# INK-USC/RE-Net

Measured on NVIDIA H100. Metric: rgcn_aggregate_edge_messages_per_sec, higher is better.
Workload: dtype f32

## Files before the change

renet_b200/csrc/common.cuh:

```cuda
#pragma once
#include <cuda_runtime.h>
#include <stdint.h>
#include <stdio.h>
#include <stdarg.h>

#include "../../include/renet_b200.h"

namespace renet {

void set_error(const char* fmt, ...);
void count_launch(int n = 1);
void note_gemm_kernel(int kernel);
int last_gemm_kernel();

#define RENET_CHECK_ARG(cond, ...)                  \
  do {                                              \
    if (!(cond)) {                                  \
      ::renet::set_error(__VA_ARGS__);              \
      return RENET_ERR_INVALID_ARG;                 \
    }                                               \
  } while (0)

#define RENET_CHECK_CUDA(expr)                                                        \
  do {                                                                                \
    cudaError_t _e = (expr);                                                          \
    if (_e != cudaSuccess) {                                                          \
      ::renet::set_error("%s failed: %s (%s:%d)", #expr, cudaGetErrorString(_e),     \
                         __FILE__, __LINE__);                                         \
      return RENET_ERR_CUDA;                                                          \
    }                                                                                 \
  } while (0)

#define RENET_CHECK_LAUNCH(name)                                                      \
  do {                                                                                \
    cudaError_t _e = cudaGetLastError();                                              \
    if (_e != cudaSuccess) {                                                          \
      ::renet::set_error("launch of %s failed: %s", name, cudaGetErrorString(_e));    \
      return RENET_ERR_CUDA;                                                          \
    }                                                                                 \
    ::renet::count_launch();                                                          \
  } while (0)

constexpr int kNumSMs = 132;

__device__ __forceinline__ float4 ldg_f4(const float* p) {
  return __ldg(reinterpret_cast<const float4*>(p));
}
__device__ __forceinline__ float4 ldg_f4_stream(const float* p) {
  float4 r;
  asm volatile("ld.global.nc.L1::no_allocate.v4.f32 {%0,%1,%2,%3}, [%4];"
               : "=f"(r.x), "=f"(r.y), "=f"(r.z), "=f"(r.w)
               : "l"(p));
  return r;
}
__device__ __forceinline__ void st_f4(float* p, float4 v) { *reinterpret_cast<float4*>(p) = v; }

__device__ __forceinline__ void red_add_f4(float* p, float4 v) {
  asm volatile("red.global.add.v4.f32 [%0], {%1,%2,%3,%4};" ::"l"(p), "f"(v.x), "f"(v.y), "f"(v.z),
               "f"(v.w)
               : "memory");
}

bool deterministic();
int set_deterministic(int on);
int det_scratch(int64_t bytes, cudaStream_t stream, void** out);
int launch_sum_partials(const float* parts, int n_parts, int64_t stride, int64_t rows, int cols, float* out, int64_t ldo,
                        bool accumulate, cudaStream_t stream);
int scatter_add_rows_det(const float* src, int64_t ld, const int32_t* index, const int32_t* outer, float* dst, int64_t n_rows,
                         int d, cudaStream_t stream);

int sgemm_nn(const float* A, const int32_t* a_index, int64_t lda, const float* B, int64_t ldb, float* C,
             int64_t ldc, const float* bias, int64_t M, int32_t N, int32_t K, bool accumulate,
             cudaStream_t stream);
bool sgemm_nn_tiled_ok(const float* A, int64_t lda, const float* B, int64_t ldb, const float* C, int64_t ldc,
                       const float* bias, int32_t N, int32_t K);
int sgemm_nn_ffma(const float* A, const int32_t* a_index, int64_t lda, const float* B, int64_t ldb, float* C,
// ... 67 lines not shown
```

renet_b200/csrc/rgcn_fwd.cu:

```cuda
#include <stdlib.h>

#include "common.cuh"
#include "rgcn_tile.cuh"
#include "rgcn_stream.cuh"

namespace renet {
namespace {

template <bool RELU, bool HAS_LOOP, bool INDEXED, int NODES = kTileNodes>
__global__ void __launch_bounds__(kTileWarps * 32, 768 / (kTileWarps * 32))
rgcn_gather_d200_kernel(const float* __restrict__ H, const int32_t* __restrict__ h_index,
                        const float* __restrict__ W, const int32_t* __restrict__ row_ptr,
                        const int32_t* __restrict__ col_src, const int32_t* __restrict__ col_type,
                        const float* __restrict__ norm, float* __restrict__ Hout, int N, int passthrough) {
  __shared__ __align__(16) float agg[NODES][200];
  __shared__ __align__(16) float loopbuf[HAS_LOOP ? NODES : 1][200];
  __shared__ __align__(16) float head[kTileWarps][200];
  __shared__ int head_mask[NODES];
  __shared__ float normbuf[NODES];
  __shared__ int s_rp[NODES + 1];
  const int tid = threadIdx.x;
  const int v0 = blockIdx.x * NODES;
  const int nv = min(NODES, N - v0);
  tile_prefetch_epilogue(loopbuf, normbuf, Hout + (int64_t)v0 * 200, norm + v0, nv, HAS_LOOP, tid, kTileWarps * 32);
// ... 65 lines not shown
    else if (e && e[0] == 's') v = 3;
  }
  return v;
}
bool gather_use_stream(int64_t E, int64_t N, bool indexed_input) {
  const int c = gather_kernel_choice();
  const int64_t min_nodes = indexed_input ? kStreamMinNodes : kStreamMinPlainNodes;
  return c == 3 || (c == 0 && E >= kStreamMinEdges && N >= min_nodes && N <= kStreamMaxNodes);
}

static long long* g_stream_dbg = nullptr;
void set_stream_debug_buffer(long long* p) { g_stream_dbg = p; }

int stream_cfg_choice() {
  static int v = -1;
  if (v < 0) {
    const char* e = getenv("RENET_STREAM_CFG");
    v = e ? atoi(e) : 0;
  }
  return v;
}

template <bool RELU, bool HAS_LOOP, bool INDEXED, class Cfg>
static int launch_stream_cfg(const float* H, const int32_t* h_index, const float* W, const int32_t* row_ptr,
                             const int32_t* col_src, const int32_t* col_type, const float* norm, float* Hout, int N, int R2,
                             const int32_t* hot_rel, int n_hot, int E_hint, cudaStream_t stream) {
  static bool attr_done = false;
  if (!attr_done) {
    RENET_CHECK_CUDA(cudaFuncSetAttribute(rgcn_gather_stream_kernel<RELU, HAS_LOOP, INDEXED, false, Cfg>,
                                          cudaFuncAttributeMaxDynamicSharedMemorySize, Cfg::kSmemBytes));
    attr_done = true;
  }
  long long* dbg = g_stream_dbg;
  rgcn_gather_stream_kernel<RELU, HAS_LOOP, INDEXED, false, Cfg><<<kNumSMs, Cfg::kThreads, Cfg::kSmemBytes, stream>>>(
      H, h_index, W, row_ptr, col_src, col_type, norm, Hout, N, R2, hot_rel, n_hot, E_hint, dbg);
  RENET_CHECK_LAUNCH("rgcn_gather_stream_kernel");
  return RENET_OK;
}

template <bool RELU, bool HAS_LOOP, bool INDEXED>
static int launch_stream(const float* H, const int32_t* h_index, const float* W, const int32_t* row_ptr,
                         const int32_t* col_src, const int32_t* col_type, const float* norm, float* Hout, int N, int R2,
                         const int32_t* hot_rel, int n_hot, int E_hint, cudaStream_t stream) {
#define RENET_ST(...) return launch_stream_cfg<RELU, HAS_LOOP, INDEXED, __VA_ARGS__>(H, h_index, W, row_ptr, col_src, col_type, norm, Hout, N, R2, hot_rel, n_hot, E_hint, stream)
  if (RELU && HAS_LOOP) {
    switch (stream_cfg_choice()) {
      case 1: RENET_ST(StCfg<28, 2, 31, false>);
      case 2: RENET_ST(StCfg<24, 2, 44, false>);
      default: break;
    }
  }
  RENET_ST(StDefault<false>);
#undef RENET_ST
}

int launch_rgcn_gather(const float* H, const int32_t* h_index, const float* W, const int32_t* row_ptr,
                       const int32_t* col_src, const int32_t* col_type, const float* norm, float* Hout,
                       int64_t N, int64_t E, int d_in, int d_out, int nb, int relu, int has_loop,
                       cudaStream_t stream, int R2, const int32_t* hot_rel, int n_hot) {
  if (N == 0) return RENET_OK;
  const int passthrough = (E == 0) ? 1 : 0;
  const bool fast = d_in == 200 && d_out == 200 && nb == 100 &&
                    ((reinterpret_cast<uintptr_t>(H) | reinterpret_cast<uintptr_t>(W) |
                      reinterpret_cast<uintptr_t>(Hout)) & 15) == 0;
  if (fast) {
    const int key = (relu ? 4 : 0) | (has_loop ? 2 : 0) | (h_index ? 1 : 0);
    if (!passthrough && gather_use_stream(E, N, h_index != nullptr)) {
#define RENET_LAUNCH_STREAM(R, L, I) return launch_stream<R, L, I>(H, h_index, W, row_ptr, col_src, col_type, norm, Hout, (int)N, R2, hot_rel, n_hot, (int)E, stream)
      switch (key) {
        case 0: RENET_LAUNCH_STREAM(false, false, false);
// ... 37 lines not shown
```

renet_b200/csrc/rgcn_stream.cuh:

```cuda
#pragma once
#include <type_traits>

#include "common.cuh"
#include "umma.cuh"

namespace renet {

constexpr int kStRpCap = 1024;
constexpr int kStMaxR2 = 2048;
constexpr int kStNodeCost = 2;
constexpr int kStSlot = 800;
constexpr int kStHotGroups = 8;
template <int WARPS, int D, int HOT, bool BWD>
struct StCfg {
  static constexpr int kWarps = WARPS, kThreads = WARPS * 32, kD = D, kHot = HOT;
  static constexpr int kHotPerGroup = (HOT + kStHotGroups - 1) / kStHotGroups;
  static constexpr int kBlk = (32 / D) * D;
  static constexpr int kOffRing = 0;
  static constexpr int kOffHot = kOffRing + WARPS * D * kStSlot;
  static constexpr int kOffHeads = kOffHot + HOT * 1600;
  static constexpr int kOffRp = kOffHeads + WARPS * 800;
  static constexpr int kOffSlotOf = kOffRp + kStRpCap * 4;
  static constexpr int kOffIdx = kOffSlotOf + kStMaxR2;
  static constexpr int kOffSc = kOffIdx + WARPS * 64 * 8;
// ... 87 lines not shown
  auto global_timer = []() {
    long long t;
    asm volatile("mov.u64 %0, %%globaltimer;" : "=l"(t));
    return t;
  };
  if (dbg) { stamp(0, clock64()); stamp(5, global_timer()); }
  constexpr int D = Cfg::kD, kBlk = Cfg::kBlk, kStWarps = Cfg::kWarps, kStThreads = Cfg::kThreads;
  float* heads = reinterpret_cast<float*>(st_smem + Cfg::kOffHeads);
  int32_t* s_rp = reinterpret_cast<int32_t*>(st_smem + Cfg::kOffRp);
  uint8_t* slot_of = st_smem + Cfg::kOffSlotOf;
  int* flags = reinterpret_cast<int*>(st_smem + Cfg::kOffFlags);
  int* s_part = flags + kStWarps;
  int* s_e0 = s_part + 16;
  uint64_t* bars = reinterpret_cast<uint64_t*>(st_smem + Cfg::kOffBars);
  int* cnt = reinterpret_cast<int*>(st_smem + Cfg::kOffRing);
  int* hist = cnt + kStMaxR2;

  const int tid = threadIdx.x, lane = tid & 31;
  const int warp = __shfl_sync(0xffffffffu, tid >> 5, 0);
  const bool tail4 = lane < 4;
  const bool use_hot = R2 > 0 && R2 <= kStMaxR2 && Cfg::kHot > 0;
  const bool given_hot = use_hot && hot_rel != nullptr;
  {
    const int64_t gt = (int64_t)blockIdx.x * Cfg::kThreads + threadIdx.x;
    const int64_t n_rp_lines = ((int64_t)N + 1 + 31) / 32, n_e_lines = ((int64_t)E_hint + 31) / 32;
    const char* pf = nullptr;
    if (gt < n_rp_lines) pf = reinterpret_cast<const char*>(row_ptr) + gt * 128;
    else if (gt < n_rp_lines + n_e_lines) pf = reinterpret_cast<const char*>(col_a) + (gt - n_rp_lines) * 128;
    else if (gt < n_rp_lines + 2 * n_e_lines) pf = reinterpret_cast<const char*>(col_type) + (gt - n_rp_lines - n_e_lines) * 128;
    else if (INDEXED && gt < 2 * n_rp_lines + 2 * n_e_lines - 1)
      pf = reinterpret_cast<const char*>(x_index) + (gt - n_rp_lines - 2 * n_e_lines) * 128;
    if (pf) asm volatile("prefetch.global.L2 [%0];" ::"l"(pf));
  }
  const int E = __ldg(row_ptr + N);
  const int half = tid >> 8, ht = tid & 255;
  const int c_idx = blockIdx.x + half;
  const bool searching = tid < 512 && c_idx > 0 && c_idx < (int)gridDim.x;
  const int probe0 = min((ht + 1) * (N / 256 + 1) - 1, N);
  const int val0 = searching ? __ldg(row_ptr + probe0) : 0;
  constexpr int kHotIters = (Cfg::kHot + 31) / 32;
  const int n_hot_given = given_hot ? min(n_hot_arg, Cfg::kHot) : 0;
  if (warp == 1) {
    for (int sl = lane; sl < n_hot_given; sl += 32) st_cp_async4(smem_u32(hist + sl), hot_rel + sl);
    asm volatile("cp.async.commit_group;" ::: "memory");
  }
  const uint32_t hot_bar0 = smem_u32(bars + kStWarps * D);
  const uint32_t head_bar0 = hot_bar0 + kStHotGroups * 8;

  if (tid < 16) s_part[tid] = 0;
  if (tid < kStWarps) flags[tid] = 0;
  if (lane == 0) {
#pragma unroll
    for (int k = 0; k < D; ++k) mbar_init(smem_u32(bars + warp * D + k), 1);
    mbar_init(head_bar0 + warp * 8, 1);
    if (warp == 0)
      for (int gr = 0; gr < kStHotGroups; ++gr) mbar_init(hot_bar0 + gr * 8, 1);
    asm volatile("fence.mbarrier_init.release.cluster;" ::: "memory");
  }
  if (!given_hot)
    for (int i = tid; i < kStMaxR2 + 256; i += kStThreads) cnt[i] = 0;
  for (int i = tid; i < kStMaxR2 / 4; i += kStThreads) reinterpret_cast<uint32_t*>(slot_of)[i] = 0u;
  __syncthreads();
  auto load_hot = [&](int n_hot, auto row_of) {
    if (lane < kStHotGroups) {
      const int rows = min(max(n_hot - lane * Cfg::kHotPerGroup, 0), Cfg::kHotPerGroup);
      st_expect_tx(hot_bar0 + lane * 8, (uint32_t)rows * 1600u);
    }
    __syncwarp();
#pragma unroll
    for (int k = 0; k < kHotIters; ++k) {
      const int sl = lane + 32 * k;
      if (sl < n_hot)
        st_bulk_g2s(smem_u32(st_smem + Cfg::kOffHot + sl * 1600), W + (int64_t)row_of(k) * 400, 1600,
                    hot_bar0 + (sl / Cfg::kHotPerGroup) * 8);
    }
  };
  const int64_t total_cost = (int64_t)E + (int64_t)kStNodeCost * N;
  const int64_t target = ((int64_t)c_idx * total_cost) / gridDim.x;
  int lo = 0, hi = N;
  const int rounds = N < 256 ? 1 : (N < 65536 ? 2 : (N < (1 << 24) ? 3 : 4));
  for (int r = 0; r < rounds; ++r) {
    const int step = (hi - lo) / 256 + 1;
    const int p = min(lo + (ht + 1) * step - 1, hi);
    const int val = r == 0 ? val0 : (searching ? __ldg(row_ptr + p) : 0);
    const bool below = searching && (int64_t)val + (int64_t)kStNodeCost * p < target;
    const unsigned m = __ballot_sync(0xffffffffu, below);
    if (lane == 0 && m) atomicAdd(&s_part[2 * r + (half & 1)], __popc(m));
    __syncthreads();
    const int f = s_part[2 * r + (half & 1)];
    if (r == rounds - 1 && searching) {
      if (ht == f) { s_part[10 + half] = lo + f; s_part[12 + half] = val; }
      if (ht == f - 1) s_part[14 + half] = val + 1;
    }
    const int new_hi = min(lo + (f + 1) * step - 1, hi);
// ... 109 lines not shown
        const int slot = atomicAdd(&s_part[9], 1);
        slot_of[r] = (uint8_t)(slot + 1);
        hist[slot] = r;
      }
    }
    __syncthreads();
    if (thr > 1) {
      for (int r = tid; r < R2; r += kStThreads) {
        if (min(cnt[r], 255) == thr - 1) {
          const int slot = atomicAdd(&s_part[9], 1);
          if (slot < Cfg::kHot) { slot_of[r] = (uint8_t)(slot + 1); hist[slot] = r; }
        }
      }
      __syncthreads();
    }
    if (warp == 1) load_hot(min(s_part[9], Cfg::kHot), [&](int k) { return hist[lane + 32 * k]; });
  }
  block_gather(0);
  __syncthreads();
  block_stage(0);
  block_load(1);

  const uint32_t ring = st_opaque(smem_u32(st_smem + Cfg::kOffRing + warp * D * kStSlot));
  const uint32_t bar0 = st_opaque(smem_u32(bars + warp * D));
  const uint32_t idx_a = st_opaque(smem_u32(my_idx));
  auto issue = [&](int k, int slot) {
    if (st_elect_one()) {
      const uint32_t src = st_lds_u32(idx_a + (((uint32_t)k & 63u) << 3));
      const uint32_t bar = bar0 + slot * 8;
      st_expect_tx(bar, 800u);
      st_bulk_g2s(ring + slot * kStSlot, X + (int64_t)(int)src * 200, 800, bar);
    }
  };
  asm volatile("griddepcontrol.wait;" ::: "memory");
#pragma unroll
  for (int k = 0; k < D; ++k)
    if (k < n) issue(k, k);

  int va;
  {
    int l = A, h = A_next;
    while (h > l) {
      const int mid = (l + h) >> 1;
      if (rp(mid) >= e0) h = mid; else l = mid + 1;
    }
    va = l;
  }
  int cur = va;
  bool continued = false;
  if (n > 0 && rp(va) > e0) { cur = va - 1; continued = true; }
  int cur_end = cur < A_next ? rp(cur + 1) : ce;
  float acc[8];
#pragma unroll
  for (int i = 0; i < 8; ++i) acc[i] = 0.f;
  float2 lp[4];
  float nrm = 1.f;
#pragma unroll
  for (int k = 0; k < 4; ++k) lp[k] = make_float2(0.f, 0.f);
  auto fetch_dest = [&](int v) {
    if (v < A_next) {
      if (HAS_LOOP) {
#pragma unroll
        for (int k = 0; k < 4; ++k)
          if (k < 3 || tail4) lp[k] = *reinterpret_cast<const float2*>(Hout + (int64_t)v * 200 + 2 * (lane + 32 * k));
      }
      if (!BWD) nrm = __ldg(norm + v);
    }
// ... 148 lines not shown
```

renet_b200/csrc/umma_gemm.cu:

```cuda
#include "common.cuh"
#include <mutex>
#include <vector>

#include "umma.cuh"

namespace renet {
namespace {

constexpr int UM = 128;
constexpr int UN = 200;
constexpr int UNP = 208;
constexpr int UKC = 40;
constexpr int USLABS = UKC / 4;
constexpr int UTHREADS = 256;
constexpr int A_SLAB_BYTES = UM * 16;
constexpr int B_SLAB_BYTES = UNP * 16;
constexpr int A_BYTES = USLABS * A_SLAB_BYTES;
constexpr int B_BYTES = USLABS * B_SLAB_BYTES;
constexpr int STAGE_BYTES = 2 * A_BYTES + 2 * B_BYTES;
constexpr int NUM_STAGES = 2;
constexpr int SMEM_BYTES = NUM_STAGES * STAGE_BYTES;
constexpr int CLD = UNP + 4;
static_assert(UM * CLD * 4 <= SMEM_BYTES, "accumulator tile reuses the operand stages");

// ... 119 lines not shown
          o[4] += b1.x; o[5] += b1.y; o[6] += b1.z; o[7] += b1.w;
        }
        if (accumulate) {
          const float4 c0 = *reinterpret_cast<const float4*>(cp), c1 = *reinterpret_cast<const float4*>(cp + 4);
          o[0] += c0.x; o[1] += c0.y; o[2] += c0.z; o[3] += c0.w;
          o[4] += c1.x; o[5] += c1.y; o[6] += c1.z; o[7] += c1.w;
        }
        st_f4(cp, make_float4(o[0], o[1], o[2], o[3]));
        st_f4(cp + 4, make_float4(o[4], o[5], o[6], o[7]));
      }
    }
  }
}


constexpr int P_BK = 32;
constexpr int P_A_BYTES = UM * 128;
constexpr int P_B_BYTES = UNP * 128;
constexpr int P_B_CHUNK = 2 * P_B_BYTES;
constexpr int P_UN = UNP / 2;
constexpr int P_BH_BYTES = P_UN * 128;
constexpr int P_STAGE = 2 * P_A_BYTES + 2 * P_BH_BYTES;
constexpr int P_THREADS = 384;
constexpr int P_CLD = P_UN + 4;
__host__ __device__ constexpr int p_stages(int epi) { return epi == 0 ? 3 : 2; }
__host__ __device__ constexpr int p_staging_bytes(int epi) { return epi == 0 ? 0 : 2 * 64 * P_CLD * 4; }
__host__ __device__ constexpr int p_smem(int epi) { return p_stages(epi) * P_STAGE + p_staging_bytes(epi) + 1024 + 128; }
static_assert(p_smem(0) <= 232448 && p_smem(1) <= 232448, "one CTA's shared memory");
static_assert(P_STAGE % 1024 == 0 && P_BH_BYTES % 1024 == 0, "swizzle atoms stay 1024-byte aligned");

__global__ void __launch_bounds__(256)
umma_pack_b_kernel(const float* __restrict__ B, int64_t sk, int64_t sn, int N, int K, uint8_t* __restrict__ Bp,
                   int n_chunks, int tile_offset) {
  const int nt = blockIdx.x, kc = blockIdx.y;
  const int n0 = nt * UN, k0 = kc * P_BK;
  const int tile_n = min(UN, N - n0);
  uint8_t* dst = Bp + (size_t)((nt + tile_offset) * n_chunks + kc) * P_B_CHUNK;
  for (int task = blockIdx.z * 256 + threadIdx.x; task < UNP * 8; task += 256 * gridDim.z) {
    const int j = task / UNP, n = task % UNP;
    float v[4];
#pragma unroll
    for (int i = 0; i < 4; ++i) {
      const int k = k0 + 4 * j + i;
      v[i] = (n < tile_n && k < K) ? __ldg(B + (int64_t)k * sk + (int64_t)(n0 + n) * sn) : 0.f;
    }
    float4 hi, lo;
    split4(make_float4(v[0], v[1], v[2], v[3]), hi, lo);
    const uint32_t off = sw128_offset(n, j);
    *reinterpret_cast<float4*>(dst + off) = hi;
    *reinterpret_cast<float4*>(dst + P_B_BYTES + off) = lo;
  }
}

struct PUnit {
  int64_t row_base;
  int nt, half, zb, split, c_begin, n_local;
};
__device__ __forceinline__ PUnit p_unit(int64_t u, int64_t n_rt, int n_tiles, int n_chunks, int k_splits) {
  PUnit w;
  const int64_t rest = u / n_rt;
  w.row_base = (u - rest * n_rt) * UM;
  const int nh = (int)(rest % (2 * n_tiles)), z = (int)(rest / (2 * n_tiles));
  w.nt = nh >> 1;
  w.half = nh & 1;
  w.zb = z / k_splits;
  w.split = z - w.zb * k_splits;
// ... 352 lines not shown
      if (n_gt) atomicAdd(rc, n_gt);
      if (n_eq) atomicAdd(rc + 1, n_eq);
#pragma unroll
      for (int j = 0; j < 2; ++j)
        if (j < n_lists) {
          if (m_gt[j]) atomicAdd(rc + 2 + 2 * j, m_gt[j]);
          if (m_eq[j]) atomicAdd(rc + 3 + 2 * j, m_eq[j]);
        }
    }
    if (FWD && gr < M) {
      const int64_t pi = (int64_t)(w.nt * 2 + w.half) * M + gr;
      epi.pmax[pi] = run_m;
      epi.psum[pi] = run_s;
      if (SOFT) {
        epi.pdot[pi] = run_pz;
        epi.pmass[pi] = run_p;
      }
    }
  }
  ts.finish(1);
}

constexpr int R_MAX_CHUNKS = 7;
constexpr int R_CHUNK = 2 * P_BH_BYTES;
constexpr int R_THREADS = 384;
constexpr int R_SMEM = R_MAX_CHUNKS * R_CHUNK + 1024 + 8 * R_MAX_CHUNKS;
static_assert(R_SMEM <= 232448, "one CTA's shared memory");

template <bool INDEXED>
__global__ void __launch_bounds__(R_THREADS, 1)
umma_gemm_resident_kernel(const float* __restrict__ A, const int32_t* __restrict__ a_index, int64_t lda,
                          const uint8_t* __restrict__ Bp, float* __restrict__ C, int64_t ldc, const float* __restrict__ bias,
                          int64_t M, const int32_t* __restrict__ m_dev, int N, int K, int n_chunks, int accumulate,
                          int64_t batch_a, int64_t batch_bp, int64_t batch_c, int n_panels, long long* dbg) {
  extern __shared__ uint8_t smem_raw[];
  const uint32_t raw = smem_u32(smem_raw);
  const uint32_t sb = raw + ((1024 - (raw & 1023)) & 1023);
  const uint32_t bar0 = sb + R_MAX_CHUNKS * R_CHUNK;
  const int tid = threadIdx.x;
  const int wg = __shfl_sync(0xffffffffu, tid >> 7, 0);
  if (m_dev != nullptr) M = *m_dev;
  const int G = gridDim.x, b = blockIdx.x;
  const int p = (int)(((int64_t)(b + 1) * n_panels - 1) / G);
  const int cta0 = (int)((int64_t)p * G / n_panels), ncta = (int)((int64_t)(p + 1) * G / n_panels) - cta0;
  const int64_t n_rt = (M + 63) / 64;
  const int64_t t_begin = (int64_t)(b - cta0) * n_rt / ncta, t_end = (int64_t)(b - cta0 + 1) * n_rt / ncta;
  if (t_begin == t_end) return;
  const int n_tiles = (N + UN - 1) / UN;
  const int half = p & 1, nt = (p >> 1) % n_tiles, zb = (p >> 1) / n_tiles;
  GemmStamps ts(dbg, wg);
  if (tid == 0) {
    for (int c = 0; c < n_chunks; ++c) mbar_init(bar0 + 8 * c, 1);
    asm volatile("fence.mbarrier_init.release.cluster;" ::: "memory");
    const uint8_t* src = Bp + zb * batch_bp + (size_t)nt * n_chunks * P_B_CHUNK + half * P_BH_BYTES;
    for (int c = 0; c < n_chunks; ++c) {
      const uint32_t bar = bar0 + 8 * c, dst = sb + c * R_CHUNK;
      mbar_expect_tx(bar, R_CHUNK);
      bulk_copy_g2s(dst, src + (size_t)c * P_B_CHUNK, P_BH_BYTES, bar);
      bulk_copy_g2s(dst + P_BH_BYTES, src + (size_t)c * P_B_CHUNK + P_B_BYTES, P_BH_BYTES, bar);
      mbar_arrive(bar);
    }
  }
  __syncthreads();

  const int wt = tid & 127, lane = tid & 31, tig = lane & 3;
  const int ra = 16 * (wt >> 5) + (lane >> 2);
  const float* Az = A + zb * batch_a;
  auto row_ptr = [&](int64_t gr) -> const float* {
    return gr < M ? Az + (INDEXED ? (int64_t)__ldg(a_index + gr) : gr) * lda : nullptr;
  };
  auto load = [&](float (&v)[16], const float* pa, const float* pb, int c) {
#pragma unroll
    for (int j = 0; j < 8; ++j) {
      const int k = c * P_BK + 4 * j + tig;
      v[j] = (pa != nullptr && k < K) ? __ldg(pa + k) : 0.f;
      v[8 + j] = (pb != nullptr && k < K) ? __ldg(pb + k) : 0.f;
    }
  };
  int64_t t = t_begin + wg;
  const float *pa = nullptr, *pb = nullptr;
  float v[16];
  if (t < t_end) {
    pa = row_ptr(t * 64 + ra);
    pb = row_ptr(t * 64 + ra + 8);
    load(v, pa, pb, 0);
  }
  const int n0 = nt * UN, cb = half * P_UN, tile_n = min(UN, N - n0);
  float* Cz = C + zb * batch_c;
  const float* bz = bias != nullptr ? bias + zb * (int64_t)N : nullptr;
  float acc[P_UN / 2];
  for (; t < t_end; t += 3) {
    ++ts.items;
    for (int c = 0; c < n_chunks; ++c) {
      long long t0 = ts.now();
      uint32_t hi[16], lo[16];
// ... 19 lines not shown
      const uint32_t b_hi = sb + c * R_CHUNK, b_lo = b_hi + P_BH_BYTES;
      wgmma_fence();
#pragma unroll
      for (int ks = 0; ks < P_BK / 8; ++ks) {
        if (ks < nks) {
          const uint64_t dBh = make_desc_sw128(b_hi + ks * 32), dBl = make_desc_sw128(b_lo + ks * 32);
          const int j = 2 * ks;
          wgmma_tf32_n104_rs(acc, hi[j], hi[8 + j], hi[j + 1], hi[9 + j], dBh, (c | ks) != 0);
          wgmma_tf32_n104_rs(acc, lo[j], lo[8 + j], lo[j + 1], lo[9 + j], dBh, 1);
          wgmma_tf32_n104_rs(acc, hi[j], hi[8 + j], hi[j + 1], hi[9 + j], dBl, 1);
        }
      }
      wgmma_commit();
      t0 = ts.now();
      wgmma_wait<0>();
      ts.mma += ts.now() - t0;
      acc_fence(acc);
      reg_fence(hi);
      reg_fence(lo);
    }
    const long long t0 = ts.now();
    store_fragment(acc, Cz, ldc, bz, t * 64, M, n0, cb, tile_n, accumulate, wt);
    ts.epi += ts.now() - t0;
  }
  ts.finish(2);
}

__device__ __forceinline__ uint32_t dedup_hash(uint32_t v, int bits) { return (v * 0x9E3779B1u) >> (32 - bits); }

__global__ void __launch_bounds__(256)
dedup_insert_kernel(const int32_t* __restrict__ a_index, int64_t M, unsigned long long* __restrict__ table, int bits,
                    uint32_t epoch, int32_t* __restrict__ slot_row, int32_t* __restrict__ uniq, int32_t* __restrict__ link,
                    int32_t* __restrict__ count) {
  const int64_t n = (int64_t)blockIdx.x * blockDim.x + threadIdx.x;
  if (n >= M) return;
  const uint32_t v = (uint32_t)__ldg(a_index + n);
  const unsigned long long key = ((unsigned long long)epoch << 32) | v;
  const uint32_t mask = (1u << bits) - 1;
  uint32_t s = dedup_hash(v, bits);
  for (;;) {
    const unsigned long long cur = __ldcg(table + s);
    if (cur == key) break;
    if ((uint32_t)(cur >> 32) == epoch) {
      s = (s + 1) & mask;
      continue;
    }
    if (atomicCAS(table + s, cur, key) == cur) {
      const int32_t u = atomicAdd(count, 1);
      uniq[u] = (int32_t)v;
      slot_row[s] = u;
      break;
    }
  }
  link[n] = (int32_t)s;
}

__global__ void __launch_bounds__(256)
dedup_expand_kernel(const float* __restrict__ P, const int32_t* __restrict__ slot_row, const int32_t* __restrict__ link,
                    float* __restrict__ C, int64_t ldc, int64_t M, int N, int32_t* __restrict__ count) {
  if (blockIdx.x == 0 && threadIdx.x == 0) *count = 0;
  const int64_t n = ((int64_t)blockIdx.x * blockDim.x + threadIdx.x) >> 5;
  if (n >= M) return;
  const int64_t u = __ldg(slot_row + __ldg(link + n));
  const float* src = P + u * N;
  float* dst = C + n * ldc;
  for (int j = 4 * (threadIdx.x & 31); j < N; j += 128) st_f4(dst + j, ldg_f4(src + j));
// ... 30 lines not shown
  *hit = false;
  std::lock_guard<std::mutex> lk(g_pack_mu);
  if (g_weight_generation < 0 || nkeys > 6) return nullptr;
  int dev = 0;
  if (cudaGetDevice(&dev) != cudaSuccess) return nullptr;
  for (auto& e : g_pack_entries) {
    if (e.device != dev || e.nkeys != nkeys || e.bytes != bytes) continue;
    bool same = true;
    for (int i = 0; i < nkeys; ++i) same &= e.keys[i] == keys[i];
    if (!same) continue;
    *hit = e.gen == g_weight_generation;
    e.gen = g_weight_generation;
    return e.buf;
  }
  if (g_pack_entries.size() >= 64) {
    cudaFree(g_pack_entries.front().buf);
    g_pack_entries.erase(g_pack_entries.begin());
  }
  PackEntry e{};
  e.device = dev; e.nkeys = nkeys; e.bytes = bytes; e.gen = g_weight_generation;
  for (int i = 0; i < nkeys; ++i) e.keys[i] = keys[i];
  if (cudaMalloc(&e.buf, (size_t)bytes) != cudaSuccess) { cudaGetLastError(); return nullptr; }
  g_pack_entries.push_back(e);
  return e.buf;
}

int64_t umma_packed_bytes(int N, int K) {
  return (int64_t)((N + UN - 1) / UN) * ((K + P_BK - 1) / P_BK) * P_B_CHUNK;
}
bool umma_shape_ok(int N, int K) { return (K % 4 == 0) && (N % 8 == 0) && N > 0 && K > 0; }

int umma_pack_b(const float* B, int64_t sk, int64_t sn, int N, int K, void* Bp, int tile_offset, cudaStream_t stream) {
  const int n_tiles = (N + UN - 1) / UN, n_chunks = (K + P_BK - 1) / P_BK;
  umma_pack_b_kernel<<<dim3(n_tiles, n_chunks, 7), 256, 0, stream>>>(B, sk, sn, N, K, (uint8_t*)Bp, n_chunks, tile_offset);
  RENET_CHECK_LAUNCH("umma_pack_b_kernel");
  return RENET_OK;
}

static bool resident_ok(int N, int K, int batch) {
  return (K + P_BK - 1) / P_BK <= R_MAX_CHUNKS && batch * ((N + UN - 1) / UN) * 2 <= kNumSMs;
}

static int launch_resident(const float* A, const int32_t* a_index, int64_t lda, const void* Bp, float* C, int64_t ldc,
                           const float* bias, int64_t M, const int32_t* m_dev, int N, int K, bool accumulate, int batch,
                           int64_t batch_a, int64_t batch_bp, int64_t batch_c, cudaStream_t stream) {
  static bool attr_r = false;
  if (!attr_r) {
    RENET_CHECK_CUDA(cudaFuncSetAttribute(umma_gemm_resident_kernel<true>, cudaFuncAttributeMaxDynamicSharedMemorySize, R_SMEM));
    RENET_CHECK_CUDA(cudaFuncSetAttribute(umma_gemm_resident_kernel<false>, cudaFuncAttributeMaxDynamicSharedMemorySize, R_SMEM));
    attr_r = true;
  }
  const int n_chunks = (K + P_BK - 1) / P_BK, n_panels = batch * ((N + UN - 1) / UN) * 2;
  const int64_t n_work = (int64_t)n_panels * ((M + 63) / 64);
  const unsigned grid = (unsigned)(n_work < kNumSMs ? n_work : kNumSMs);
  if (a_index)
    umma_gemm_resident_kernel<true><<<grid, R_THREADS, R_SMEM, stream>>>(A, a_index, lda, (const uint8_t*)Bp, C, ldc, bias, M,
                                                                        m_dev, N, K, n_chunks, accumulate, batch_a, batch_bp,
                                                                        batch_c, n_panels, g_gemm_dbg);
  else
    umma_gemm_resident_kernel<false><<<grid, R_THREADS, R_SMEM, stream>>>(A, a_index, lda, (const uint8_t*)Bp, C, ldc, bias, M,
                                                                         m_dev, N, K, n_chunks, accumulate, batch_a, batch_bp,
                                                                         batch_c, n_panels, g_gemm_dbg);
  RENET_CHECK_LAUNCH("umma_gemm_resident_kernel");
  note_gemm_kernel(RENET_GEMM_RESIDENT);
  return RENET_OK;
}

static int launch_streaming(const float* A, const int32_t* a_index, int64_t lda, const void* Bp, float* C, int64_t ldc,
                            const float* bias, int64_t M, int N, int K, bool accumulate, int batch, int64_t batch_a,
                            int64_t batch_bp, int64_t batch_c, int epi_mode, const EpiArgs& epi, int k_splits, int64_t split_c,
                            cudaStream_t stream) {
  static bool attr2 = false;
  if (!attr2) {
    RENET_CHECK_CUDA(cudaFuncSetAttribute(umma_gemm_packed_kernel<true, 0>, cudaFuncAttributeMaxDynamicSharedMemorySize, p_smem(0)));
    RENET_CHECK_CUDA(cudaFuncSetAttribute(umma_gemm_packed_kernel<false, 0>, cudaFuncAttributeMaxDynamicSharedMemorySize, p_smem(0)));
    RENET_CHECK_CUDA(cudaFuncSetAttribute(umma_gemm_packed_kernel<false, 1>, cudaFuncAttributeMaxDynamicSharedMemorySize, p_smem(1)));
    RENET_CHECK_CUDA(cudaFuncSetAttribute(umma_gemm_packed_kernel<false, 2>, cudaFuncAttributeMaxDynamicSharedMemorySize, p_smem(2)));
    RENET_CHECK_CUDA(cudaFuncSetAttribute(umma_gemm_packed_kernel<false, 3>, cudaFuncAttributeMaxDynamicSharedMemorySize, p_smem(3)));
    RENET_CHECK_CUDA(cudaFuncSetAttribute(umma_gemm_packed_kernel<false, 4>, cudaFuncAttributeMaxDynamicSharedMemorySize, p_smem(4)));
    RENET_CHECK_CUDA(cudaFuncSetAttribute(umma_gemm_packed_kernel<false, 5>, cudaFuncAttributeMaxDynamicSharedMemorySize, p_smem(5)));
    RENET_CHECK_CUDA(cudaFuncSetAttribute(umma_gemm_packed_kernel<false, 6>, cudaFuncAttributeMaxDynamicSharedMemorySize, p_smem(6)));
    RENET_CHECK_CUDA(cudaFuncSetAttribute(umma_gemm_packed_kernel<false, 7>, cudaFuncAttributeMaxDynamicSharedMemorySize, p_smem(7)));
    attr2 = true;
  }
  const int n_tiles = (N + UN - 1) / UN, n_chunks = (K + P_BK - 1) / P_BK;
  const int64_t n_units = (M + UM - 1) / UM * (2 * n_tiles) * batch * k_splits;
  const unsigned grid = (unsigned)(n_units < kNumSMs ? n_units : kNumSMs);
#define RENET_UMMA_LAUNCH(IDX, EP)                                                                                       \
  umma_gemm_packed_kernel<IDX, EP><<<grid, P_THREADS, p_smem(EP), stream>>>(A, a_index, lda, (const uint8_t*)Bp, C, ldc, bias, \
                                                                           M, N, K, n_chunks, accumulate, batch_a, batch_bp,  \
                                                                           batch_c, epi, k_splits, split_c, n_units, \
                                                                           g_gemm_dbg)
  if (epi_mode == 1) RENET_UMMA_LAUNCH(false, 1);
  else if (epi_mode == 2) RENET_UMMA_LAUNCH(false, 2);
  else if (epi_mode == 3) RENET_UMMA_LAUNCH(false, 3);
  else if (epi_mode == 4) RENET_UMMA_LAUNCH(false, 4);
// ... 84 lines not shown
  }
  if (M > w->rows) {
    if (w->ix) RENET_CHECK_CUDA(cudaFreeAsync(w->ix, stream));
    w->ix = nullptr;
    w->rows = w->slots = 0;
    int64_t s = 1;
    while (s < 2 * rows) s <<= 1;
    const size_t bytes = (size_t)s * 12 + (size_t)rows * 8 + 16;
    RENET_CHECK_CUDA(cudaMallocAsync((void**)&w->ix, bytes, stream));
    RENET_CHECK_CUDA(cudaMemsetAsync(w->ix, 0, bytes, stream));
    w->rows = rows;
    w->slots = s;
  }
  if (++w->epoch == 0) {
    RENET_CHECK_CUDA(cudaMemsetAsync(w->ix, 0, (size_t)w->slots * 8, stream));
    w->epoch = 1;
  }
  *out = *w;
  return RENET_OK;
}

static int umma_gemm_dedup(const float* A, const int32_t* a_index, int64_t lda, const void* Bp, float* C, int64_t ldc,
                           const float* bias, int64_t M, int N, int K, cudaStream_t stream) {
  DedupWs w;
  int rc = dedup_workspace(M, N, stream, &w);
  if (rc) return rc;
  int bits = 1;
  while ((int64_t(1) << bits) < 2 * M) ++bits;
  unsigned long long* table = reinterpret_cast<unsigned long long*>(w.ix);
  int32_t* slot_row = reinterpret_cast<int32_t*>(w.ix + w.slots * 8);
  int32_t* uniq = slot_row + w.slots;
  int32_t* link = uniq + w.rows;
  int32_t* count = link + w.rows;
  dedup_insert_kernel<<<(unsigned)((M + 255) / 256), 256, 0, stream>>>(a_index, M, table, bits, w.epoch, slot_row, uniq, link,
                                                                       count);
  RENET_CHECK_LAUNCH("dedup_insert_kernel");
  if ((rc = launch_resident(A, uniq, lda, Bp, w.P, N, bias, M, count, N, K, false, 1, 0, 0, 0, stream))) return rc;
  dedup_expand_kernel<<<(unsigned)((M + 7) / 8), 256, 0, stream>>>(w.P, slot_row, link, C, ldc, M, N, count);
  RENET_CHECK_LAUNCH("dedup_expand_kernel");
  note_gemm_kernel(RENET_GEMM_DEDUP);
  return RENET_OK;
}

int umma_gemm_prepacked_ex(const float* A, const int32_t* a_index, int64_t lda, const void* Bp, float* C, int64_t ldc,
                           const float* bias, int64_t M, int N, int K, bool accumulate, int batch, int64_t batch_a,
                           int64_t batch_bp, int64_t batch_c, int epi_mode, const EpiArgs& epi, int k_splits, int64_t split_c,
                           cudaStream_t stream) {
  if (M <= 0) return RENET_OK;
  const int n_chunks = (K + P_BK - 1) / P_BK;
  if (k_splits < 1) k_splits = 1;
  if (k_splits > n_chunks) k_splits = n_chunks;
  while (k_splits > 1 && ((n_chunks + k_splits - 1) / k_splits) * (k_splits - 1) >= n_chunks) --k_splits;
  if (epi_mode == 0 && k_splits == 1 && resident_ok(N, K, batch)) {
    const int rc = launch_resident(A, a_index, lda, Bp, C, ldc, bias, M, nullptr, N, K, accumulate, batch, batch_a, batch_bp,
                                   batch_c, stream);
    return rc ? rc : 1;
  }
  const int rc = launch_streaming(A, a_index, lda, Bp, C, ldc, bias, M, N, K, accumulate, batch, batch_a, batch_bp, batch_c,
                                  epi_mode, epi, k_splits, split_c, stream);
  return rc ? rc : k_splits;
}

int umma_gemm_prepacked(const float* A, const int32_t* a_index, int64_t lda, const void* Bp, float* C, int64_t ldc,
                        const float* bias, int64_t M, int N, int K, bool accumulate, int batch, int64_t batch_a,
                        int64_t batch_bp, int64_t batch_c, cudaStream_t stream) {
  EpiArgs none{};
  const int r = umma_gemm_prepacked_ex(A, a_index, lda, Bp, C, ldc, bias, M, N, K, accumulate, batch, batch_a, batch_bp, batch_c,
                                       0, none, 1, 0, stream);
  return r < 0 ? r : RENET_OK;
}

int umma_gemm_nn_try(const float* A, const int32_t* a_index, int64_t lda, const float* B, int64_t ldb, float* C,
                     int64_t ldc, const float* bias, int64_t M, int32_t N, int32_t K, bool accumulate,
                     cudaStream_t stream) {
  const bool aligned = ((reinterpret_cast<uintptr_t>(A) | reinterpret_cast<uintptr_t>(B) | reinterpret_cast<uintptr_t>(C) |
                         reinterpret_cast<uintptr_t>(bias)) & 15) == 0;
  if (aligned && umma_shape_ok(N, K) && (lda % 4 == 0) && (ldc % 4 == 0) && M >= 64 && g_scratch != nullptr &&
      umma_packed_bytes(N, K) <= g_scratch_bytes && (reinterpret_cast<uintptr_t>(g_scratch) & 127) == 0) {
    bool hit = false;
    const void* keys[4] = {B, reinterpret_cast<const void*>((intptr_t)ldb), reinterpret_cast<const void*>((intptr_t)N),
                           reinterpret_cast<const void*>((intptr_t)K)};
    void* cached = packed_cache_lookup(keys, 4, umma_packed_bytes(N, K), &hit);
    void* Bp = cached ? cached : g_scratch;
    int rc = hit ? 0 : umma_pack_b(B, ldb, 1, N, K, Bp, 0, stream);
    if (rc) return rc;
    if (a_index != nullptr && !accumulate && M >= kDedupMinRows && resident_ok(N, K, 1))
      rc = umma_gemm_dedup(A, a_index, lda, Bp, C, ldc, bias, M, N, K, stream);
    else
      rc = umma_gemm_prepacked(A, a_index, lda, Bp, C, ldc, bias, M, N, K, accumulate, 1, 0, 0, 0, stream);
    return rc ? rc : 1;
  }
  if (M < 64 || !legacy_ok(A, lda, B, ldb, C, ldc, bias, N, K)) return 0;
  const int rc = launch_legacy(A, a_index, lda, B, ldb, C, ldc, bias, M, N, K, accumulate, stream);
  return rc ? rc : 1;
}

int debug_gemm(int form, int kernel, const float* A, const int32_t* a_index, int64_t lda, const float* B, int64_t ldb, float* C,
               int64_t ldc, const float* bias, int64_t M, int N, int64_t K, bool accumulate, int batch, int64_t batch_a,
               int64_t batch_b, int64_t batch_c, void* ws, int64_t ws_bytes, cudaStream_t stream) {
  RENET_CHECK_ARG(form >= RENET_GEMM_FORM_NN && form <= RENET_GEMM_FORM_TN, "renet_debug_gemm: unknown form %d", form);
  RENET_CHECK_ARG(kernel >= 0 && kernel <= RENET_GEMM_DEDUP, "renet_debug_gemm: unknown kernel %d", kernel);
  RENET_CHECK_ARG(M >= 0 && N > 0 && K > 0 && K < (int64_t(1) << 31) && lda > 0 && ldb > 0 && ldc > 0 && batch >= 1 &&
                      (batch == 1 || form == RENET_GEMM_FORM_PREPACKED),
                  "renet_debug_gemm: bad shape");
  RENET_CHECK_ARG(A && B && C, "renet_debug_gemm: null pointer");
  const bool ffma = kernel == RENET_GEMM_FFMA_TILED || kernel == RENET_GEMM_FFMA_NAIVE;
  if (form == RENET_GEMM_FORM_TN) {
    RENET_CHECK_ARG(kernel == 0 || ffma, "renet_debug_gemm: the tn form runs on the FFMA kernels only");
    RENET_CHECK_ARG(M < (int64_t(1) << 31) && bias == nullptr, "renet_debug_gemm: the tn form takes M < 2^31 and no bias");
    RENET_CHECK_ARG(kernel != RENET_GEMM_FFMA_TILED || sgemm_tn_tiled_ok(A, lda, B, ldb, C, ldc, (int)M, N),
                    "renet_debug_gemm: the tiled tn kernel needs 16-byte aligned operands and M, N, ld* multiples of 4");
    if (M == 0) return RENET_OK;
    return sgemm_tn(A, a_index, lda, B, ldb, C, ldc, (int)M, N, K, accumulate, stream, kernel == RENET_GEMM_FFMA_NAIVE);
  }
  if (form == RENET_GEMM_FORM_NN && (kernel == 0 || ffma || kernel == RENET_GEMM_LEGACY)) {
    RENET_CHECK_ARG(kernel != RENET_GEMM_FFMA_TILED || sgemm_nn_tiled_ok(A, lda, B, ldb, C, ldc, bias, N, (int)K),
                    "renet_debug_gemm: the tiled FFMA kernel needs 16-byte aligned operands and N, K, ld* multiples of 4");
    RENET_CHECK_ARG(kernel != RENET_GEMM_LEGACY || legacy_ok(A, lda, B, ldb, C, ldc, bias, N, (int)K),
                    "renet_debug_gemm: the legacy kernel needs K %% 40 == 0, N %% 8 == 0, ld* %% 4 == 0, 16-byte aligned operands");
    if (M == 0) return RENET_OK;
    if (kernel == 0) return sgemm_nn(A, a_index, lda, B, ldb, C, ldc, bias, M, N, (int)K, accumulate, stream);
    if (ffma) return sgemm_nn_ffma(A, a_index, lda, B, ldb, C, ldc, bias, M, N, (int)K, accumulate,
                                   kernel == RENET_GEMM_FFMA_NAIVE, stream);
    return launch_legacy(A, a_index, lda, B, ldb, C, ldc, bias, M, N, (int)K, accumulate, stream);
  }
  RENET_CHECK_ARG(kernel == 0 || kernel == RENET_GEMM_STREAMING || kernel == RENET_GEMM_RESIDENT ||
                      (kernel == RENET_GEMM_DEDUP && form == RENET_GEMM_FORM_NN),
                  "renet_debug_gemm: kernel %d cannot serve form %d", kernel, form);
  const bool aligned = ((reinterpret_cast<uintptr_t>(A) | reinterpret_cast<uintptr_t>(C) | reinterpret_cast<uintptr_t>(bias)) &
                        15) == 0;
  RENET_CHECK_ARG(aligned && umma_shape_ok(N, (int)K) && lda % 4 == 0 && ldc % 4 == 0 && batch_a % 4 == 0 && batch_c % 4 == 0,
                  "renet_debug_gemm: the packed kernels need 16-byte aligned A / C / bias, K %% 4 == 0, N %% 8 == 0 and "
                  "lda, ldc, batch strides multiples of 4");
  RENET_CHECK_ARG((kernel != RENET_GEMM_RESIDENT && kernel != RENET_GEMM_DEDUP) || resident_ok(N, (int)K, batch),
                  "renet_debug_gemm: the resident kernel needs K <= %d and at most %d panels", R_MAX_CHUNKS * P_BK, kNumSMs);
  RENET_CHECK_ARG(kernel != RENET_GEMM_DEDUP || (a_index != nullptr && !accumulate),
                  "renet_debug_gemm: the deduplicated product needs an index and no accumulate");
  const int64_t pb = umma_packed_bytes(N, (int)K);
  RENET_CHECK_ARG(ws != nullptr && ws_bytes >= batch * pb && (reinterpret_cast<uintptr_t>(ws) & 127) == 0,
                  "renet_debug_gemm: the workspace needs %lld bytes, 128-byte aligned", (long long)(batch * pb));
  if (M == 0) return RENET_OK;
  for (int b = 0; b < batch; ++b) {
    const int rc = umma_pack_b(B + b * batch_b, ldb, 1, N, (int)K, static_cast<uint8_t*>(ws) + b * pb, 0, stream);
    if (rc) return rc;
  }
  if (kernel == RENET_GEMM_DEDUP) return umma_gemm_dedup(A, a_index, lda, ws, C, ldc, bias, M, N, (int)K, stream);
  if (kernel == RENET_GEMM_RESIDENT)
    return launch_resident(A, a_index, lda, ws, C, ldc, bias, M, nullptr, N, (int)K, accumulate, batch, batch_a, pb, batch_c,
                           stream);
  if (kernel == RENET_GEMM_STREAMING)
    return launch_streaming(A, a_index, lda, ws, C, ldc, bias, M, N, (int)K, accumulate, batch, batch_a, pb, batch_c, 0,
                            EpiArgs{}, 1, 0, stream);
  return umma_gemm_prepacked(A, a_index, lda, ws, C, ldc, bias, M, N, (int)K, accumulate, batch, batch_a, pb, batch_c, stream);
}

}
```

Baseline: 2.629 billion.

## Chain kernels with programmatic dependent launch and overlap prologues with predecessors

```diff
diff --git a/renet_b200/csrc/common.cuh b/renet_b200/csrc/common.cuh
--- a/renet_b200/csrc/common.cuh
+++ b/renet_b200/csrc/common.cuh
@@ -42,6 +42,32 @@
   } while (0)
 
 constexpr int kNumSMs = 132;
+
+__device__ __forceinline__ void pdl_wait() { asm volatile("griddepcontrol.wait;" ::: "memory"); }
+__device__ __forceinline__ void pdl_trigger() { asm volatile("griddepcontrol.launch_dependents;" ::: "memory"); }
+
+template <class... KArgs, class... Args>
+int launch_chained(const char* name, void (*kernel)(KArgs...), dim3 grid, dim3 block, size_t smem, cudaStream_t stream,
+                   Args&&... args) {
+  cudaLaunchAttribute attr[1];
+  attr[0].id = cudaLaunchAttributeProgrammaticStreamSerialization;
+  attr[0].val.programmaticStreamSerializationAllowed = 1;
+  cudaLaunchConfig_t cfg = {};
+  cfg.gridDim = grid;
+  cfg.blockDim = block;
+  cfg.dynamicSmemBytes = smem;
+  cfg.stream = stream;
+  cfg.attrs = attr;
+  cfg.numAttrs = 1;
+  const cudaError_t e = cudaLaunchKernelEx(&cfg, kernel, static_cast<KArgs>(args)...);
+  if (e != cudaSuccess) {
+    cudaGetLastError();
+    set_error("launch of %s failed: %s", name, cudaGetErrorString(e));
+    return RENET_ERR_CUDA;
+  }
+  count_launch();
+  return RENET_OK;
+}
 
 __device__ __forceinline__ float4 ldg_f4(const float* p) {
   return __ldg(reinterpret_cast<const float4*>(p));
diff --git a/renet_b200/csrc/rgcn_fwd.cu b/renet_b200/csrc/rgcn_fwd.cu
--- a/renet_b200/csrc/rgcn_fwd.cu
+++ b/renet_b200/csrc/rgcn_fwd.cu
@@ -121,10 +121,9 @@
     attr_done = true;
   }
   long long* dbg = g_stream_dbg;
-  rgcn_gather_stream_kernel<RELU, HAS_LOOP, INDEXED, false, Cfg><<<kNumSMs, Cfg::kThreads, Cfg::kSmemBytes, stream>>>(
-      H, h_index, W, row_ptr, col_src, col_type, norm, Hout, N, R2, hot_rel, n_hot, E_hint, dbg);
-  RENET_CHECK_LAUNCH("rgcn_gather_stream_kernel");
-  return RENET_OK;
+  return launch_chained("rgcn_gather_stream_kernel", rgcn_gather_stream_kernel<RELU, HAS_LOOP, INDEXED, false, Cfg>,
+                        dim3(kNumSMs), dim3(Cfg::kThreads), Cfg::kSmemBytes, stream, H, h_index, W, row_ptr, col_src, col_type,
+                        norm, Hout, N, R2, hot_rel, n_hot, E_hint, dbg);
 }
 
 template <bool RELU, bool HAS_LOOP, bool INDEXED>
diff --git a/renet_b200/csrc/rgcn_stream.cuh b/renet_b200/csrc/rgcn_stream.cuh
--- a/renet_b200/csrc/rgcn_stream.cuh
+++ b/renet_b200/csrc/rgcn_stream.cuh
@@ -143,6 +143,24 @@
       pf = reinterpret_cast<const char*>(x_index) + (gt - n_rp_lines - 2 * n_e_lines) * 128;
     if (pf) asm volatile("prefetch.global.L2 [%0];" ::"l"(pf));
   }
+  const uint32_t hot_bar0 = smem_u32(bars + kStWarps * D);
+  const uint32_t head_bar0 = hot_bar0 + kStHotGroups * 8;
+
+  if (tid < 16) s_part[tid] = 0;
+  if (tid < kStWarps) flags[tid] = 0;
+  if (lane == 0) {
+#pragma unroll
+    for (int k = 0; k < D; ++k) mbar_init(smem_u32(bars + warp * D + k), 1);
+    mbar_init(head_bar0 + warp * 8, 1);
+    if (warp == 0)
+      for (int gr = 0; gr < kStHotGroups; ++gr) mbar_init(hot_bar0 + gr * 8, 1);
+    asm volatile("fence.mbarrier_init.release.cluster;" ::: "memory");
+  }
+  if (!given_hot)
+    for (int i = tid; i < kStMaxR2 + 256; i += kStThreads) cnt[i] = 0;
+  for (int i = tid; i < kStMaxR2 / 4; i += kStThreads) reinterpret_cast<uint32_t*>(slot_of)[i] = 0u;
+  pdl_wait();
+  pdl_trigger();
   const int E = __ldg(row_ptr + N);
   const int half = tid >> 8, ht = tid & 255;
   const int c_idx = blockIdx.x + half;
@@ -155,22 +173,6 @@
     for (int sl = lane; sl < n_hot_given; sl += 32) st_cp_async4(smem_u32(hist + sl), hot_rel + sl);
     asm volatile("cp.async.commit_group;" ::: "memory");
   }
-  const uint32_t hot_bar0 = smem_u32(bars + kStWarps * D);
-  const uint32_t head_bar0 = hot_bar0 + kStHotGroups * 8;
-
-  if (tid < 16) s_part[tid] = 0;
-  if (tid < kStWarps) flags[tid] = 0;
-  if (lane == 0) {
-#pragma unroll
-    for (int k = 0; k < D; ++k) mbar_init(smem_u32(bars + warp * D + k), 1);
-    mbar_init(head_bar0 + warp * 8, 1);
-    if (warp == 0)
-      for (int gr = 0; gr < kStHotGroups; ++gr) mbar_init(hot_bar0 + gr * 8, 1);
-    asm volatile("fence.mbarrier_init.release.cluster;" ::: "memory");
-  }
-  if (!given_hot)
-    for (int i = tid; i < kStMaxR2 + 256; i += kStThreads) cnt[i] = 0;
-  for (int i = tid; i < kStMaxR2 / 4; i += kStThreads) reinterpret_cast<uint32_t*>(slot_of)[i] = 0u;
   __syncthreads();
   auto load_hot = [&](int n_hot, auto row_of) {
     if (lane < kStHotGroups) {
@@ -346,7 +348,6 @@
       st_bulk_g2s(ring + slot * kStSlot, X + (int64_t)(int)src * 200, 800, bar);
     }
   };
-  asm volatile("griddepcontrol.wait;" ::: "memory");
 #pragma unroll
   for (int k = 0; k < D; ++k)
     if (k < n) issue(k, k);
diff --git a/renet_b200/csrc/umma_gemm.cu b/renet_b200/csrc/umma_gemm.cu
--- a/renet_b200/csrc/umma_gemm.cu
+++ b/renet_b200/csrc/umma_gemm.cu
@@ -175,6 +175,8 @@
 __global__ void __launch_bounds__(256)
 umma_pack_b_kernel(const float* __restrict__ B, int64_t sk, int64_t sn, int N, int K, uint8_t* __restrict__ Bp,
                    int n_chunks, int tile_offset) {
+  pdl_wait();
+  pdl_trigger();
   const int nt = blockIdx.x, kc = blockIdx.y;
   const int n0 = nt * UN, k0 = kc * P_BK;
   const int tile_n = min(UN, N - n0);
@@ -593,26 +595,21 @@
 umma_gemm_resident_kernel(const float* __restrict__ A, const int32_t* __restrict__ a_index, int64_t lda,
                           const uint8_t* __restrict__ Bp, float* __restrict__ C, int64_t ldc, const float* __restrict__ bias,
                           int64_t M, const int32_t* __restrict__ m_dev, int N, int K, int n_chunks, int accumulate,
-                          int64_t batch_a, int64_t batch_bp, int64_t batch_c, int n_panels, long long* dbg) {
+                          int64_t batch_a, int64_t batch_bp, int64_t batch_c, int n_panels, int b_after_wait, long long* dbg) {
   extern __shared__ uint8_t smem_raw[];
   const uint32_t raw = smem_u32(smem_raw);
   const uint32_t sb = raw + ((1024 - (raw & 1023)) & 1023);
   const uint32_t bar0 = sb + R_MAX_CHUNKS * R_CHUNK;
   const int tid = threadIdx.x;
   const int wg = __shfl_sync(0xffffffffu, tid >> 7, 0);
-  if (m_dev != nullptr) M = *m_dev;
   const int G = gridDim.x, b = blockIdx.x;
   const int p = (int)(((int64_t)(b + 1) * n_panels - 1) / G);
   const int cta0 = (int)((int64_t)p * G / n_panels), ncta = (int)((int64_t)(p + 1) * G / n_panels) - cta0;
-  const int64_t n_rt = (M + 63) / 64;
-  const int64_t t_begin = (int64_t)(b - cta0) * n_rt / ncta, t_end = (int64_t)(b - cta0 + 1) * n_rt / ncta;
-  if (t_begin == t_end) return;
   const int n_tiles = (N + UN - 1) / UN;
   const int half = p & 1, nt = (p >> 1) % n_tiles, zb = (p >> 1) / n_tiles;
-  GemmStamps ts(dbg, wg);
-  if (tid == 0) {
-    for (int c = 0; c < n_chunks; ++c) mbar_init(bar0 + 8 * c, 1);
-    asm volatile("fence.mbarrier_init.release.cluster;" ::: "memory");
+  const bool pre = !b_after_wait && (m_dev != nullptr || (int64_t)(b - cta0) * ((M + 63) / 64) / ncta !=
+                                                             (int64_t)(b - cta0 + 1) * ((M + 63) / 64) / ncta);
+  auto issue_panel = [&]() {
     const uint8_t* src = Bp + zb * batch_bp + (size_t)nt * n_chunks * P_B_CHUNK + half * P_BH_BYTES;
     for (int c = 0; c < n_chunks; ++c) {
       const uint32_t bar = bar0 + 8 * c, dst = sb + c * R_CHUNK;
@@ -621,7 +618,24 @@
       bulk_copy_g2s(dst + P_BH_BYTES, src + (size_t)c * P_B_CHUNK + P_B_BYTES, P_BH_BYTES, bar);
       mbar_arrive(bar);
     }
-  }
+  };
+  if (tid == 0) {
+    for (int c = 0; c < n_chunks; ++c) mbar_init(bar0 + 8 * c, 1);
+    asm volatile("fence.mbarrier_init.release.cluster;" ::: "memory");
+    if (pre) issue_panel();
+  }
+  pdl_wait();
+  pdl_trigger();
+  if (m_dev != nullptr) M = *m_dev;
+  const int64_t n_rt = (M + 63) / 64;
+  const int64_t t_begin = (int64_t)(b - cta0) * n_rt / ncta, t_end = (int64_t)(b - cta0 + 1) * n_rt / ncta;
+  if (t_begin == t_end) {
+    if (pre && tid == 0)
+      for (int c = 0; c < n_chunks; ++c) mbar_wait(bar0 + 8 * c, 0);
+    return;
+  }
+  GemmStamps ts(dbg, wg);
+  if (tid == 0 && !pre) issue_panel();
   __syncthreads();
 
   const int wt = tid & 127, lane = tid & 31, tig = lane & 3;
@@ -707,6 +721,8 @@
 dedup_insert_kernel(const int32_t* __restrict__ a_index, int64_t M, unsigned long long* __restrict__ table, int bits,
                     uint32_t epoch, int32_t* __restrict__ slot_row, int32_t* __restrict__ uniq, int32_t* __restrict__ link,
                     int32_t* __restrict__ count) {
+  pdl_wait();
+  pdl_trigger();
   const int64_t n = (int64_t)blockIdx.x * blockDim.x + threadIdx.x;
   if (n >= M) return;
   const uint32_t v = (uint32_t)__ldg(a_index + n);
@@ -803,9 +819,8 @@
 
 int umma_pack_b(const float* B, int64_t sk, int64_t sn, int N, int K, void* Bp, int tile_offset, cudaStream_t stream) {
   const int n_tiles = (N + UN - 1) / UN, n_chunks = (K + P_BK - 1) / P_BK;
-  umma_pack_b_kernel<<<dim3(n_tiles, n_chunks, 7), 256, 0, stream>>>(B, sk, sn, N, K, (uint8_t*)Bp, n_chunks, tile_offset);
-  RENET_CHECK_LAUNCH("umma_pack_b_kernel");
-  return RENET_OK;
+  return launch_chained("umma_pack_b_kernel", umma_pack_b_kernel, dim3(n_tiles, n_chunks, 7), dim3(256), 0, stream, B, sk, sn, N,
+                        K, (uint8_t*)Bp, n_chunks, tile_offset);
 }
 
 static bool resident_ok(int N, int K, int batch) {
@@ -814,7 +829,7 @@
 
 static int launch_resident(const float* A, const int32_t* a_index, int64_t lda, const void* Bp, float* C, int64_t ldc,
                            const float* bias, int64_t M, const int32_t* m_dev, int N, int K, bool accumulate, int batch,
-                           int64_t batch_a, int64_t batch_bp, int64_t batch_c, cudaStream_t stream) {
+                           int64_t batch_a, int64_t batch_bp, int64_t batch_c, bool b_after_wait, cudaStream_t stream) {
   static bool attr_r = false;
   if (!attr_r) {
     RENET_CHECK_CUDA(cudaFuncSetAttribute(umma_gemm_resident_kernel<true>, cudaFuncAttributeMaxDynamicSharedMemorySize, R_SMEM));
@@ -824,15 +839,12 @@
   const int n_chunks = (K + P_BK - 1) / P_BK, n_panels = batch * ((N + UN - 1) / UN) * 2;
   const int64_t n_work = (int64_t)n_panels * ((M + 63) / 64);
   const unsigned grid = (unsigned)(n_work < kNumSMs ? n_work : kNumSMs);
-  if (a_index)
-    umma_gemm_resident_kernel<true><<<grid, R_THREADS, R_SMEM, stream>>>(A, a_index, lda, (const uint8_t*)Bp, C, ldc, bias, M,
-                                                                        m_dev, N, K, n_chunks, accumulate, batch_a, batch_bp,
-                                                                        batch_c, n_panels, g_gemm_dbg);
-  else
-    umma_gemm_resident_kernel<false><<<grid, R_THREADS, R_SMEM, stream>>>(A, a_index, lda, (const uint8_t*)Bp, C, ldc, bias, M,
-                                                                         m_dev, N, K, n_chunks, accumulate, batch_a, batch_bp,
-                                                                         batch_c, n_panels, g_gemm_dbg);
-  RENET_CHECK_LAUNCH("umma_gemm_resident_kernel");
+  const int rc = launch_chained("umma_gemm_resident_kernel",
+                                a_index ? umma_gemm_resident_kernel<true> : umma_gemm_resident_kernel<false>, dim3(grid),
+                                dim3(R_THREADS), R_SMEM, stream, A, a_index, lda, (const uint8_t*)Bp, C, ldc, bias, M, m_dev, N,
+                                K, n_chunks, (int)accumulate, batch_a, batch_bp, batch_c, n_panels, (int)b_after_wait,
+                                g_gemm_dbg);
+  if (rc) return rc;
   note_gemm_kernel(RENET_GEMM_RESIDENT);
   return RENET_OK;
 }
@@ -983,10 +995,10 @@
   int32_t* uniq = slot_row + w.slots;
   int32_t* link = uniq + w.rows;
   int32_t* count = link + w.rows;
-  dedup_insert_kernel<<<(unsigned)((M + 255) / 256), 256, 0, stream>>>(a_index, M, table, bits, w.epoch, slot_row, uniq, link,
-                                                                       count);
-  RENET_CHECK_LAUNCH("dedup_insert_kernel");
-  if ((rc = launch_resident(A, uniq, lda, Bp, w.P, N, bias, M, count, N, K, false, 1, 0, 0, 0, stream))) return rc;
+  if ((rc = launch_chained("dedup_insert_kernel", dedup_insert_kernel, dim3((unsigned)((M + 255) / 256)), dim3(256), 0, stream,
+                           a_index, M, table, bits, w.epoch, slot_row, uniq, link, count)))
+    return rc;
+  if ((rc = launch_resident(A, uniq, lda, Bp, w.P, N, bias, M, count, N, K, false, 1, 0, 0, 0, false, stream))) return rc;
   dedup_expand_kernel<<<(unsigned)((M + 7) / 8), 256, 0, stream>>>(w.P, slot_row, link, C, ldc, M, N, count);
   RENET_CHECK_LAUNCH("dedup_expand_kernel");
   note_gemm_kernel(RENET_GEMM_DEDUP);
@@ -1004,7 +1016,7 @@
   while (k_splits > 1 && ((n_chunks + k_splits - 1) / k_splits) * (k_splits - 1) >= n_chunks) --k_splits;
   if (epi_mode == 0 && k_splits == 1 && resident_ok(N, K, batch)) {
     const int rc = launch_resident(A, a_index, lda, Bp, C, ldc, bias, M, nullptr, N, K, accumulate, batch, batch_a, batch_bp,
-                                   batch_c, stream);
+                                   batch_c, true, stream);
     return rc ? rc : 1;
   }
   const int rc = launch_streaming(A, a_index, lda, Bp, C, ldc, bias, M, N, K, accumulate, batch, batch_a, batch_bp, batch_c,
@@ -1037,6 +1049,8 @@
     if (rc) return rc;
     if (a_index != nullptr && !accumulate && M >= kDedupMinRows && resident_ok(N, K, 1))
       rc = umma_gemm_dedup(A, a_index, lda, Bp, C, ldc, bias, M, N, K, stream);
+    else if (resident_ok(N, K, 1))
+      rc = launch_resident(A, a_index, lda, Bp, C, ldc, bias, M, nullptr, N, K, accumulate, 1, 0, 0, 0, !hit, stream);
     else
       rc = umma_gemm_prepacked(A, a_index, lda, Bp, C, ldc, bias, M, N, K, accumulate, 1, 0, 0, 0, stream);
     return rc ? rc : 1;
@@ -1098,7 +1112,7 @@
   if (kernel == RENET_GEMM_DEDUP) return umma_gemm_dedup(A, a_index, lda, ws, C, ldc, bias, M, N, (int)K, stream);
   if (kernel == RENET_GEMM_RESIDENT)
     return launch_resident(A, a_index, lda, ws, C, ldc, bias, M, nullptr, N, (int)K, accumulate, batch, batch_a, pb, batch_c,
-                           stream);
+                           true, stream);
   if (kernel == RENET_GEMM_STREAMING)
     return launch_streaming(A, a_index, lda, ws, C, ldc, bias, M, N, (int)K, accumulate, batch, batch_a, pb, batch_c, 0,
                             EpiArgs{}, 1, 0, stream);
```

After: 2.686 billion, median of 6. 2.2% higher.
